# AUTOMATIC1111/stable-diffusion-webui

Hardware: AMD Instinct MI355X
Metric: images/sec SD1.5 512x512 20-step Euler-a, batch 8 per GPU (higher is better)
Workload: dtype f16

## Files before the change

include/sdmi.h:

```cpp
#ifndef SDMI_H
#define SDMI_H

#include <stdint.h>

#ifdef __cplusplus
extern "C" {
#endif

#define SDMI_VERSION 100

enum { SDMI_F16 = 0, SDMI_F32 = 1 };

typedef struct sdmi_engine sdmi_engine;

int sdmi_version(void);
const char* sdmi_last_error(void);
int sdmi_device_ok(void);


int64_t sdmi_attention_workspace_bytes(int B, int H, int M, int D);
int sdmi_attention(const void* q, const void* k, const void* v, void* out,
                   int B, int H, int N, int M, int D,
                   int ldq, int ldk, int ldv, int ldo, float scale,
                   void* workspace, int64_t workspace_bytes, void* stream);

int64_t sdmi_attention_wide_workspace_bytes(int B, int N, int M, int D);
int sdmi_attention_wide(const void* q, const void* k, const void* v, void* out,
                        int B, int N, int M, int D,
                        int ldq, int ldk, int ldv, int ldo, float scale,
                        void* workspace, int64_t workspace_bytes, void* stream);

int sdmi_attention_vt(const void* q, const void* k, const void* vt, void* out,
                      int B, int H, int N, int M, int D,
                      int ldq, int ldk, int vt_ld, int ldo, float scale, int force_generic, void* stream);

typedef struct sdmi_conv_desc {
    const void* a0;
    const void* a1;
    const void* w;
    const void* bias;
    const void* rowbias;
    const void* resid;
    void* out;
    int32_t c0, c1, lda0, lda1;
    int32_t B, Hi, Wi, Ho, Wo;
    int32_t taps;
    int32_t stride;
    int32_t pad;
    int32_t up;
// ... 323 lines not shown
```

stable-diffusion-webui_amd/_lib.py:

```python
from __future__ import annotations

import ctypes as C
import os
import re

_HERE = os.path.dirname(os.path.abspath(__file__))
LIB_PATH = os.environ.get("SDMI_LIB") or os.path.join(_HERE, "lib", "libsdmi.so")
HEADER_PATH = os.path.join(os.path.dirname(_HERE), "include", "sdmi.h")

F16, F32 = 0, 1
EP_OUT_F32, EP_GEGLU, EP_NCHW, EP_BIAS_ROW = 1, 2, 4, 8
EP_TRANSPOSE = 64
EP_WRAP = 128
RRDB_EP_NONE, RRDB_EP_LRELU, RRDB_EP_RES1, RRDB_EP_RES2, RRDB_EP_RELU = 0, 1, 2, 3, 4
RRDB_ST_F16, RRDB_ST_F32_NCHW, RRDB_ST_U8_HWC = 0, 1, 2
COMPACT_EP_NONE, COMPACT_EP_PRELU, COMPACT_EP_TAIL = 0, 1, 2


class SdmiError(RuntimeError):
    pass


class ConvDesc(C.Structure):
    _fields_ = [
# ... 86 lines not shown
        f"{LIB_PATH} is missing: build it with `python -c 'import __graft_entry__ as g; g.build()'` "
        "(hipcc --offload-arch=gfx950). There is no CPU fallback for the MI355X engine.")

lib = C.CDLL(LIB_PATH)

_vp, _i, _i64, _f, _u32 = C.c_void_p, C.c_int, C.c_int64, C.c_float, C.c_uint32
_SIGS = {
    "sdmi_version": (C.c_int, []),
    "sdmi_last_error": (C.c_char_p, []),
    "sdmi_device_ok": (C.c_int, []),
    "sdmi_attention_workspace_bytes": (_i64, [_i, _i, _i, _i]),
    "sdmi_attention": (_i, [_vp, _vp, _vp, _vp, _i, _i, _i, _i, _i, _i, _i, _i, _i, _f, _vp, _i64, _vp]),
    "sdmi_attention_wide_workspace_bytes": (_i64, [_i, _i, _i, _i]),
    "sdmi_attention_wide": (_i, [_vp, _vp, _vp, _vp, _i, _i, _i, _i, _i, _i, _i, _i, _f, _vp, _i64, _vp]),
    "sdmi_attention_vt": (_i, [_vp, _vp, _vp, _vp, _i, _i, _i, _i, _i, _i, _i, _i, _i, _f, _i, _vp]),
    "sdmi_conv_gemm": (_i, [C.POINTER(ConvDesc), _vp]),
    "sdmi_conv_splitk_workspace_bytes": (_i64, [_i, _i, _i, _i]),
    "sdmi_bench_conv_gemm": (_i, [C.POINTER(ConvDesc), _i, C.POINTER(C.c_float), _vp]),
    "sdmi_pack_conv_weight": (_i, [_vp, _i, _vp, _i, _i, _i, _i, _i, _i, _i, _vp]),
    "sdmi_groupnorm": (_i, [_vp, _vp, _i, _i, _vp, _vp, _vp, _i, _i, _i, _f, _i, _vp, _i64, _vp]),
    "sdmi_groupnorm_workspace_bytes": (_i64, [_i, _i, _i]),
    "sdmi_layernorm": (_i, [_vp, _vp, _vp, _vp, _i64, _i, _f, _vp]),
    "sdmi_rowchain_ff_pack_bytes": (_i64, [_i, _i]),
    "sdmi_rowchain_ff_pack": (_i, [_vp, _vp, _vp, _vp, _i, _i, _vp]),
    "sdmi_rowchain_ff": (_i, [_vp, _vp, _vp, _vp, _vp, _vp, _i64, _i, _i, _f, _vp]),
    "sdmi_xattn_chain": (_i, [_vp, _vp, _vp, _vp, _vp, _vp, _vp, _vp, _vp, _i64, _i, _i, _i, _i, _i, _f, _vp]),
    "sdmi_philox_randn": (_i, [_vp, _i64, C.c_uint64, C.c_uint32, _vp]),
    "sdmi_slerp": (_i, [_vp, _vp, _vp, _f, _i, _i, _i, _vp, _vp]),
    "sdmi_cfg_prepare_input": (_i, [_vp, _vp, _vp, _i, _i, _i, _i64, _vp]),
    "sdmi_cfg_prepare_concat": (_i, [_vp, _vp, _vp, _vp, _i, _i, _i, _i, _i, _i64, _u32, _vp]),
# ... 120 lines not shown
```

stable-diffusion-webui_amd/csrc/attention.hip:

```cpp
#include "common.h"
#include "prof.h"
#include <cstdlib>

namespace sdmi {

typedef float f2v __attribute__((ext_vector_type(2)));
typedef unsigned u4v __attribute__((ext_vector_type(4)));

__device__ __forceinline__ float max3f(float a, float b, float c) { return fmaxf(fmaxf(a, b), c); }
template <int NKB>
__device__ __forceinline__ float tree_max(const f16v (&sc)[NKB]) {
    constexpr int N = NKB * 16;
    float v[N];
#pragma unroll
    for (int i = 0; i < N; ++i) v[i] = sc[i >> 4][i & 15];
    int n = N;
#pragma unroll
    for (int level = 0; level < 6; ++level) {
        if (n <= 1) break;
        const int m = (n + 2) / 3;
#pragma unroll
        for (int i = 0; i < m; ++i) {
            const int a = 3 * i, b = a + 1 < n ? a + 1 : a, c = a + 2 < n ? a + 2 : a;
            v[i] = max3f(v[a], v[b], v[c]);
        }
        n = m;
    }
    return v[0];
}

__device__ __forceinline__ float fold_p2(float c) { return __builtin_bit_cast(float, __builtin_bit_cast(unsigned, c) & 0x7F800000u); }

template <int D, int KVT, int VAR = 0>
__global__ __launch_bounds__(256, ((VAR == 15 || VAR == 16 || VAR == 17 || VAR == 18) ? 3 : (VAR == 5 || VAR >= 10) ? 4 : D <= 80 ? 2 : 1)) void attn_mfma_kernel(AttnP p) {
    constexpr bool LAZY_RESCALE = VAR >= 5;
    constexpr bool PREF = VAR == 15 || VAR == 16 || VAR == 17 || VAR == 18;
    constexpr bool FOLD = VAR == 17 && ((D + 15) / 16 * 16) > D;
    constexpr bool TREEMAX = VAR == 16;
    constexpr bool TIMING = VAR == 18;
    long long tm[6] = {0, 0, 0, 0, 0, 0};
    auto stamp = [&]() -> long long {
        if constexpr (!TIMING) return 0;
        const long long t = __builtin_amdgcn_s_memtime();
        asm volatile("s_waitcnt lgkmcnt(0)" ::: "memory");
        return t;
    };
    constexpr bool NO_EXP = VAR == 10, NO_S = VAR == 11, NO_PV = VAR == 12, NO_MAX = VAR == 13, NO_STAGE = VAR == 14;
    constexpr int DK = (D + 15) / 16 * 16;
    constexpr int NDC = DK / 16;
    constexpr int DV = (D + 31) / 32 * 32;
    constexpr int NDB = DV / 32;
    constexpr int NKB = KVT / 32;
// ... 24 lines not shown
            bh = blockIdx.y; qb = blockIdx.x;
        }
    }
    const int b = bh / p.H, h = bh - b * p.H;
    const int q = qb * 128 + wave * 32 + lq;
    const bool qok = q < p.N;

    h8 qf[NDC];
    {
        const half_t* qptr = p.q + ((long)b * p.N + (qok ? q : 0)) * p.ldq + h * D;
#pragma unroll
        for (int dc = 0; dc < NDC; ++dc) {
            const int d = dc * 16 + half * 8;
            h8 v = {0, 0, 0, 0, 0, 0, 0, 0};
            if (qok && d < D) v = *reinterpret_cast<const h8*>(qptr + d);
            if constexpr (FOLD) {
#pragma unroll
                for (int e = 0; e < 8; ++e) v[e] = (half_t)((float)v[e] * fold_p2(p.scale_log2));
            }
            qf[dc] = v;
        }
    }
    constexpr int F_DC = D / 16, F_HALF = (D >> 3) & 1, F_E = D & 7;
    float shift = 0.f;

    const half_t* kbase = p.k + (long)b * p.M * p.ldk + h * D;
    const half_t* vbase = p.vt + ((long)b * p.H + h) * D * (long)p.vt_ld;

    u4v kr[K_IT], vr[V_IT];
    auto load_tile = [&](int t) {
        const int key0 = t * KVT;
#pragma unroll
        for (int it = 0; it < K_IT; ++it) {
            const int idx = it * 256 + tid;
            const int row = idx / KCPR, c = idx - row * KCPR;
            const int rr = min(key0 + row, p.M - 1);
            const int cc = (DK == D || c * 8 < D) ? c : 0;
            kr[it] = *reinterpret_cast<const u4v*>(kbase + (long)rr * p.ldk + cc * 8);
        }
#pragma unroll
        for (int it = 0; it < V_IT; ++it) {
            const int idx = it * 256 + tid;
            const int row = idx / VCPR, c = idx - row * VCPR;
            int col = key0 + c * 8;
            if (KVT > 64) col = min(col, p.vt_ld - 8);
            vr[it] = *reinterpret_cast<const u4v*>(vbase + (long)min(row, D - 1) * p.vt_ld + col);
        }
    };
    auto write_tile = [&](int buf) {
        char* Ks = smem + buf * TILE_BYTES;
        char* Vs = Ks + K_BYTES;
#pragma unroll
        for (int it = 0; it < K_IT; ++it) {
            const int idx = it * 256 + tid;
            const int row = idx / KCPR, c = idx - row * KCPR;
            if ((KCH % 256 == 0 || it + 1 < K_IT || idx < KCH) && !(FOLD && c * 8 >= D)) *reinterpret_cast<u4v*>(Ks + row * KSTR + c * 16) = kr[it];
        }
#pragma unroll
        for (int it = 0; it < V_IT; ++it) {
            const int idx = it * 256 + tid;
            const int row = idx / VCPR, c = idx - row * VCPR;
// ... 28 lines not shown
        constexpr int PADCH = (DV - D) * VCPR;
        for (int i = tid; i < 2 * PADCH; i += 256) {
            const int buf = i / PADCH, j = i - buf * PADCH;
            const int row = D + j / VCPR, c = j % VCPR;
            const unsigned w = row == D ? 0x3C003C00u : 0u;
            *reinterpret_cast<uint4*>(smem + buf * TILE_BYTES + K_BYTES + row * VSTR + c * 16) = make_uint4(w, w, w, w);
        }
    }
    __syncthreads();

    const f2v sl2 = {p.scale_log2, p.scale_log2};
    for (int t = 0; t < ntiles; ++t) {
        const int cur = t & 1;
        const bool more = !NO_STAGE && t + 1 < ntiles;
        const long long ta = stamp();
        if (more) load_tile(t + 1);
        const char* tile = smem + (NO_STAGE ? 0 : cur) * TILE_BYTES;

        f16v sc[NKB];
#pragma unroll
        for (int kb = 0; kb < NKB; ++kb)
#pragma unroll
            for (int r = 0; r < 16; ++r) sc[kb][r] = 0.f;
        h8 vaf[PREF ? NDB : 1][PREF ? NKB : 1][2];
        if constexpr (PREF) {
            h8 kaf[NDC][NKB];
#pragma unroll
            for (int dc = 0; dc < NDC; ++dc)
#pragma unroll
                for (int kb = 0; kb < NKB; ++kb) kaf[dc][kb] = *reinterpret_cast<const h8*>(tile + ka_off + kb * 32 * KSTR + dc * 32);
// ... 24 lines not shown

        const long long tb = stamp();
        if (t >= nfull || p.causal) {
            asm volatile("");
            int lim = p.M - t * KVT - 8 * half;
            if (p.causal) lim = min(lim, q + 1 - t * KVT - 8 * half);
#pragma unroll
            for (int kb = 0; kb < NKB; ++kb)
#pragma unroll
                for (int r = 0; r < 16; ++r)
                    if (32 * kb + 16 * (r >> 3) + (r & 7) >= lim) sc[kb][r] = -INFINITY;
        }
        h8 pb[NKB][2];
        long long tc = 0;
        if constexpr (FOLD) {
            const float fr = p.scale_log2 / fold_p2(p.scale_log2);
            const f2v fr2 = {fr, fr};
            float mx = -INFINITY;
#pragma unroll
            for (int kb = 0; kb < NKB; ++kb)
#pragma unroll
                for (int r = 0; r < 16; ++r) mx = fmaxf(mx, sc[kb][r]);
            float mlo = mx, mhi = mx;
            asm volatile("s_nop 1\n\tv_permlane32_swap_b32 %0, %1" : "+v"(mlo), "+v"(mhi));
            mx = fmaxf(mlo, mhi);
            const bool up = t == 0 || mx * fr > fmaxf(p.tau, 0.f);
            if (__builtin_amdgcn_ballot_w64(up) != 0) {
                asm volatile("");
                const float want = fmaxf(shift + mx, -60000.f);
                half_t hs = (half_t)want;
                float f = (float)hs;
                if (f < want) {
                    unsigned short bits = __builtin_bit_cast(unsigned short, hs);
                    bits = (f >= 0.f) ? (unsigned short)(bits + 1) : (unsigned short)(bits - 1);
                    hs = __builtin_bit_cast(half_t, bits);
                    f = (float)hs;
                }
                const float delta = up ? f - shift : 0.f;
                if (up) shift = f;
                const float alpha = __builtin_amdgcn_exp2f(-delta * fr);
#pragma unroll
                for (int kb = 0; kb < NKB; ++kb)
#pragma unroll
                    for (int r = 0; r < 16; ++r) sc[kb][r] -= delta;
#pragma unroll
                for (int db = 0; db < NDB; ++db)
#pragma unroll
                    for (int r = 0; r < 16; ++r) o[db][r] *= alpha;
                if (half == F_HALF) qf[F_DC][F_E] = (half_t)(-shift);
            }
#pragma unroll
            for (int kb = 0; kb < NKB; ++kb)
#pragma unroll
                for (int r = 0; r < 16; r += 2) {
                    const f2v y = f2v{sc[kb][r], sc[kb][r + 1]} * fr2;
                    pb[kb][r >> 3][r & 7] = (half_t)__builtin_amdgcn_exp2f(y.x);
                    pb[kb][r >> 3][(r & 7) + 1] = (half_t)__builtin_amdgcn_exp2f(y.y);
                }
        } else {
        float mx = -INFINITY;
        if constexpr (NO_MAX) { mx = sc[0][0] * p.scale_log2; }
        else {
        if constexpr (TREEMAX) mx = tree_max<NKB>(sc);
        else {
#pragma unroll
        for (int kb = 0; kb < NKB; ++kb)
#pragma unroll
            for (int r = 0; r < 16; ++r) mx = fmaxf(mx, sc[kb][r]);
        }
        if constexpr (PREF) {
// ... 532 lines not shown
}

template <int D, bool FOLD, int NG = 2, bool TIMING = false>
static int launch_attn_pp(const AttnP& p, hipStream_t s) {
    constexpr int DK = (D + 15) / 16 * 16, DV = (D + 31) / 32 * 32;
    constexpr int SMEM = 3 * (64 * (DK * 2 + 16) + DV * (64 * 2 + 16)) + 64 * (DK * 2 + 16) + NG * 256 * 16;
    auto kern = attn_pp_kernel<D, FOLD, NG, TIMING>;
    static PerDeviceOnce attr;
    if (attr.need()) SDMI_CHECK_HIP(hipFuncSetAttribute((const void*)kern, hipFuncAttributeMaxDynamicSharedMemorySize, SMEM));
    dim3 grid(cdiv(p.N, NG * 128), p.B * p.H);
    hipLaunchKernelGGL(kern, grid, dim3(NG * 256), SMEM, s, p);
    SDMI_CHECK_HIP(hipGetLastError());
    return 0;
}

int launch_attention(const AttnP& p_in, bool force_generic, hipStream_t s) {
    AttnP p = p_in;
    p.tau = (float)(g_attn_tau < 0 ? -1 : g_attn_tau > 12 ? 12 : g_attn_tau);
    SDMI_REQUIRE(p.B > 0 && p.H > 0 && p.N > 0 && p.M > 0 && p.D > 0, "empty attention");
    SDMI_REQUIRE(p.vt_ld >= (p.M + 63) / 64 * 64, "vt_ld must be >= M rounded up to 64");
    const double pf_flops = 4.0 * p.B * p.H * (double)p.N * p.M * p.D;
    const double pf_bytes = 2.0 * p.B * p.H * ((double)p.N * p.D * 2 + (double)p.M * p.D * 2);
    ProfScope ps(force_generic ? "attention_generic" : (p.M > 128 ? "attention_mfma_self" : "attention_mfma_cross"), pf_flops, pf_bytes, s);
    const bool aligned = (p.ldq % 8 == 0) && (p.ldk % 8 == 0) && (p.vt_ld % 8 == 0) && (p.ldo % 4 == 0) && (p.D % 8 == 0);
    const bool kvt128 = g_attn_kvt == 128;
    if (!force_generic && aligned) {
        if (g_attn_kvt == 96 && p.M > 64 && p.M <= 96 && !p.causal) {
            switch (p.D) {
                case 40: return launch_attn_d<40, 96, 0>(p, s);
                case 64: return launch_attn_d<64, 96>(p, s);
                case 80: return launch_attn_d<80, 96>(p, s);
                case 160: return launch_attn_d<160, 96>(p, s);
                default: break;
            }
        }
        switch (p.D) {
            case 40:
                if ((g_attn_occ == 20 || g_attn_occ == 21) && p.M >= g_attn_pp_min_m && p.N >= 256)
                    return g_attn_occ == 21 ? launch_attn_pp<40, true>(p, s) : launch_attn_pp<40, false>(p, s);
                if ((g_attn_occ == 28 || g_attn_occ == 38) && p.M >= g_attn_pp_min_m && p.N >= 384) {
                    AttnP q = p; q.dbg = (long long*)g_attn_dbg;
                    return g_attn_occ == 38 ? launch_attn_pp<40, true, 3, true>(q, s) : launch_attn_pp<40, true, 2, true>(q, s);
                }
                if ((g_attn_occ == 30 || g_attn_occ == 31) && p.M >= g_attn_pp_min_m && p.N >= 384)
                    return g_attn_occ == 31 ? launch_attn_pp<40, true, 3>(p, s) : launch_attn_pp<40, false, 3>(p, s);
                if (!(kvt128 && p.M > 64)) {
                    if (g_attn_occ == 5) return launch_attn_d<40, 64, 5>(p, s);
                    if (g_attn_occ == 15 && g_attn_fold_min_m > 0 && p.M >= g_attn_fold_min_m && p.N >= g_attn_fold_min_m && !p.causal)
                        return launch_attn_d<40, 64, 17>(p, s);
                    if (g_attn_occ == 15) return launch_attn_d<40, 64, 15>(p, s);
                    if (g_attn_occ == 16) return launch_attn_d<40, 64, 16>(p, s);
                    if (g_attn_occ == 17) return launch_attn_d<40, 64, 17>(p, s);
#ifdef SDMI_ATTN_PARTS
                    if (g_attn_occ == 10) return launch_attn_d<40, 64, 10>(p, s);
                    if (g_attn_occ == 11) return launch_attn_d<40, 64, 11>(p, s);
                    if (g_attn_occ == 12) return launch_attn_d<40, 64, 12>(p, s);
                    if (g_attn_occ == 13) return launch_attn_d<40, 64, 13>(p, s);
                    if (g_attn_occ == 14) return launch_attn_d<40, 64, 14>(p, s);
                    if (g_attn_occ == 18) { AttnP q = p; q.dbg = (long long*)g_attn_dbg; return launch_attn_d<40, 64, 18>(q, s); }
#endif
                }
                return (kvt128 && p.M > 64) ? launch_attn_d<40, 128>(p, s) : launch_attn_d<40, 64>(p, s);
            case 64:
                if ((g_attn_occ == 20 || g_attn_occ == 21) && p.M >= g_attn_pp_min_m && p.N >= 256) return launch_attn_pp<64, false>(p, s);
                return (kvt128 && p.M > 64) ? launch_attn_d<64, 128>(p, s) : launch_attn_d<64, 64>(p, s);
            case 80: return launch_attn_d<80, 64>(p, s);
            case 128: return launch_attn_d<128, 64>(p, s);
            case 160: return launch_attn_d<160, 64>(p, s);
            default: break;
        }
    }
    SDMI_REQUIRE(p.D <= 512 && p.M <= 16384, "generic attention supports D <= 512 and M <= 16384");
    static PerDeviceOnce attr;
    if (attr.need()) SDMI_CHECK_HIP(hipFuncSetAttribute((const void*)attn_generic_kernel, hipFuncAttributeMaxDynamicSharedMemorySize, 16384 * 4));
    hipLaunchKernelGGL(attn_generic_kernel, dim3(p.N, p.B * p.H), dim3(64), p.M * sizeof(float), s, p);
    SDMI_CHECK_HIP(hipGetLastError());
    return 0;
}

// ... 2 lines not shown
```

stable-diffusion-webui_amd/csrc/capi.cpp:

```cpp
#include "engine.h"
#include "prof.h"
#include <cstring>

namespace sdmi {
extern int g_vae_attn_rows;
int unet_forward(sdmi_engine* e, const void* x, const void* t, const void* ctx, const void* y, void* out, int io_dtype,
                 int Bn, int h, int w, int L, hipStream_t s);
int vae_decode(sdmi_engine* e, const void* z, int io_dtype, float* out, int B, int h, int w, hipStream_t s);
int vae_encode(sdmi_engine* e, const void* x, int io_dtype, float* out, int B, int H, int W, hipStream_t s);
int engine_load_unet_tensor(sdmi_engine* e, const char* key, const void* data, int dtype, int ndim, const int64_t* shape, int on_device);
int engine_load_vae_tensor(sdmi_engine* e, const char* key, const void* data, int dtype, int ndim, const int64_t* shape, int on_device);
int engine_unet_finalize(sdmi_engine* e);
int engine_clip_configure(sdmi_engine* e, int slot, const sdmi_clip_config* cfg);
int engine_clip_load_tensor(sdmi_engine* e, int slot, const char* key, const void* data, int dtype, int ndim, const int64_t* shape, int on_device);
int engine_clip_finalize(sdmi_engine* e, int slot);
int engine_clip_forward(sdmi_engine* e, int slot, const int* tokens, const float* inputs_embeds, int B, int L, int skip,
                        int apply_final_ln, float* out, float* pooled, hipStream_t s);
int engine_unet_update_weight(sdmi_engine* e, const char* key, const void* data, int dtype, int ndim, const int64_t* shape, int on_device);
int engine_vae_finalize(sdmi_engine* e);
int engine_hypernet_clear(sdmi_engine* e);
int engine_hypernet_begin(sdmi_engine* e, float multiplier);
int engine_hypernet_linear(sdmi_engine* e, int dim, int which, const void* w, const void* b, int dtype, int out_f, int in_f, int on_device);
int engine_hypernet_act(sdmi_engine* e, int dim, int which, int act);
int engine_hypernet_layernorm(sdmi_engine* e, int dim, int which, const void* g, const void* b, int dtype, int n, int on_device);
// ... 48 lines not shown
    const int64_t mpad = (M + 63) / 64 * 64;
    return (int64_t)B * H * D * mpad * (int64_t)sizeof(half_t);
}

int sdmi_attention_vt(const void* q, const void* k, const void* vt, void* out, int B, int H, int N, int M, int D, int ldq,
                      int ldk, int vt_ld, int ldo, float scale, int force_generic, void* stream) {
    API_GUARD_BEGIN
    AttnP p{};
    p.q = (const half_t*)q; p.k = (const half_t*)k; p.vt = (const half_t*)vt; p.out = (half_t*)out;
    p.B = B; p.H = H; p.N = N; p.M = M; p.D = D; p.ldq = ldq; p.ldk = ldk; p.vt_ld = vt_ld; p.ldo = ldo;
    p.scale_log2 = scale * 1.4426950408889634f;
    return launch_attention(p, force_generic != 0, (hipStream_t)stream);
    API_GUARD_END
}

int sdmi_attention(const void* q, const void* k, const void* v, void* out, int B, int H, int N, int M, int D, int ldq,
                   int ldk, int ldv, int ldo, float scale, void* workspace, int64_t workspace_bytes, void* stream) {
    API_GUARD_BEGIN
    SDMI_REQUIRE(workspace && workspace_bytes >= sdmi_attention_workspace_bytes(B, H, M, D), "attention workspace too small");
    const int mpad = (M + 63) / 64 * 64;
    if (launch_transpose_v((const half_t*)v, (half_t*)workspace, B, H, M, D, ldv, mpad, (hipStream_t)stream)) return 1;
    return sdmi_attention_vt(q, k, workspace, out, B, H, N, M, D, ldq, ldk, mpad, ldo, scale, 0, stream);
    API_GUARD_END
}

static constexpr int kWideRows = 4096;
int64_t sdmi_attention_wide_workspace_bytes(int B, int N, int M, int D) {
    if (B <= 0 || N <= 0 || M <= 0 || D <= 0) return 0;
    const int64_t mpad = (M + 63) / 64 * 64;
    const int64_t rows = N < kWideRows ? N : kWideRows;
// ... 677 lines not shown
    else if (n == "vae_attn_rows") g_vae_attn_rows = value;
    else if (n == "gemm_shortk_maxk") g_shortk_max_k = value;
    else if (n == "gemm_geglu_cfg") g_geglu_gemm_cfg = value;
    else if (n == "vt_mode") g_vt_mode = value;
    else if (n == "tile_order") g_tile_order = value;
    else if (n == "conv_korder") g_conv_korder = value < 0 ? g_conv_korder_default : value;
    else if (n == "small_linear_lds") g_small_linear_lds = value;
    else if (n == "gn_fuse") g_gn_fuse = value;
    else if (n == "gn_small") g_gn_small = value;
    else if (n == "ep_wide") g_ep_wide = value;
    else if (n == "attn_kvt") g_attn_kvt = value;
    else if (n == "attn_occ") g_attn_occ = value;
    else if (n == "attn_lds_pad") g_attn_lds_pad = value;
    else if (n == "attn_fold_min_m") g_attn_fold_min_m = value;
    else if (n == "attn_tau") g_attn_tau = value;
    else if (n == "attn_dbg_lo") g_attn_dbg = (g_attn_dbg & 0xFFFFFFFF00000000ull) | (unsigned)value;
    else if (n == "attn_dbg_hi") g_attn_dbg = (g_attn_dbg & 0xFFFFFFFFull) | ((unsigned long long)(unsigned)value << 32);
    else if (n == "gemm_split") g_force_gemm_split = value;
    else if (n == "gemm_pipe") g_gemm_pipe = value < 0 ? g_gemm_pipe_default : value;
    else if (n == "gemm_lin") g_gemm_lin = value < 0 ? 1 : value;
    else if (n == "gn_apply_blocks") g_gn_apply_blocks = value < 0 ? 0 : value;
    else if (n == "gn_band_elems") g_gn_band_elems = value < 0 ? 0 : value;
    else if (n == "gemm_dbgflags") g_gemm_dbgflags = value & 0x1F00;
    else if (n == "gemm_dbg_lo") g_gemm_dbg = (g_gemm_dbg & 0xFFFFFFFF00000000ull) | (unsigned)value;
    else if (n == "gemm_dbg_hi") g_gemm_dbg = (g_gemm_dbg & 0xFFFFFFFFull) | ((unsigned long long)(unsigned)value << 32);
    else { set_error("unknown debug knob " + n); return 1; }
    return 0;
    API_GUARD_END
}

// ... 73 lines not shown
```

stable-diffusion-webui_amd/csrc/common.h:

```cpp
#pragma once
#include <hip/hip_runtime.h>
#include <stdint.h>
#include <string>

typedef _Float16 half_t;
typedef _Float16 h8 __attribute__((ext_vector_type(8)));
typedef _Float16 h4 __attribute__((ext_vector_type(4)));
typedef _Float16 h2 __attribute__((ext_vector_type(2)));
typedef float f4 __attribute__((ext_vector_type(4)));
typedef float f16v __attribute__((ext_vector_type(16)));

namespace sdmi {

#ifndef SDMI_GELU_SIG
#define SDMI_GELU_SIG 1
#endif
__device__ __forceinline__ float geglu_gate(float val, float g) {
    const float gc = fminf(fmaxf(g, -10.0f), 10.0f);
    const float g2 = gc * gc;
    float p = fmaf(1.01426306e-3f, g2, -0.106775724f);
    p = fmaf(p, g2, -2.30112135f);
    const float e = __builtin_amdgcn_exp2f(p * gc);
    return (val * g) * __builtin_amdgcn_rcpf(1.0f + e);
}
// ... 108 lines not shown
extern int g_conv_korder;
extern int g_conv_korder_default;
extern int g_tile_order;
extern int g_vt_mode;
extern long g_gn_band_elems;
extern int g_gn_apply_blocks;
extern int g_gemm_lin;
extern int g_gemm_pipe;
extern int g_gemm_pipe_default;
extern int g_force_gemm_split;
extern int g_attn_kvt;
extern int g_attn_occ;
extern int g_attn_lds_pad;
extern int g_attn_fold_min_m;
extern int g_attn_tau;
extern unsigned long long g_attn_dbg;
extern int g_gemm_dbgflags;
extern unsigned long long g_gemm_dbg;

struct AttnP {
    const half_t* q;
    const half_t* k;
    const half_t* vt;
    half_t* out;
    int B, H, N, M, D;
    int ldq, ldk, vt_ld, ldo;
    float scale_log2;
    int causal;
    long long* dbg;
    float tau;
};
int launch_attention(const AttnP& p, bool force_generic, hipStream_t s);
int launch_transpose_v(const half_t* v, half_t* vt, int B, int H, int M, int D, int ldv, int Mpad, hipStream_t s);

bool rowchain_supports(int C);
size_t rowchain_ff_pack_bytes(int C, int hidden);
int launch_rowchain_ff_pack(const half_t* w1, const float* b1, const half_t* w2, void* packs, int C, int hidden, bool permuted,
                            hipStream_t s);
int launch_rowchain_ff(const half_t* x, half_t* out, const float* gamma, const float* beta, const void* packs, const float* bias_out,
                       long rows, int C, int hidden, float eps, hipStream_t s);

int launch_xattn_chain(const half_t* x, half_t* out, const float* gamma, const float* beta, const half_t* wq, const half_t* wo,
                       const float* bo, const half_t* k, const half_t* vt, long rows, int rows_per_image, int C, int heads, int L, int Lpad,
                       float eps, hipStream_t s);

enum { RRDB_EP_NONE = 0, RRDB_EP_LRELU = 1,
       RRDB_EP_RES1 = 2,
// ... 154 lines not shown
```

stable-diffusion-webui_amd/csrc/engine.cpp:

```cpp
#include "engine.h"

#include <algorithm>
#include <cmath>
#include <cstring>
#include <functional>

namespace sdmi {

static thread_local std::string g_err;
void set_error(const std::string& m) { g_err = m; }
const char* get_error() { return g_err.c_str(); }

const half_t* zero_page() {
    static thread_local int cached_dev = -1;
    static thread_local half_t* cached = nullptr;
    static std::map<int, half_t*> pages;
    int dev = 0;
    if (hipGetDevice(&dev) != hipSuccess) return nullptr;
    if (dev == cached_dev) return cached;
    auto it = pages.find(dev);
    if (it == pages.end()) {
        void* p = nullptr;
        if (hipMalloc(&p, kZeroPageHalfs * sizeof(half_t)) != hipSuccess) return nullptr;
        if (hipMemset(p, 0, kZeroPageHalfs * sizeof(half_t)) != hipSuccess) return nullptr;
// ... 511 lines not shown
        ConvArgs c;
        c.a0 = t2; c.c0 = w.cout; c.B = B; c.Hi = H; c.Wi = Wd; c.Ho = H; c.Wo = Wd; c.pad = 1;
        c.resid = resid; c.ldr = w.cout; c.out = o; c.ldo = w.cout;
        c.resid_lo = resid_lo; c.out_lo = acc ? r.lo(o, (out_buf ? LR : M) * w.cout) : nullptr;
        c.alpha = ss; c.bias_scale = ss;
        c.stats_C = ss == 1.f ? w.cout : 0;
        c.stats_ws_pre = st_pre;
        TRY(run_conv(r, w.c2, c));
    }
    if (reuse) r.ar->rewind(mk);
    *out = o;
    return 0;
}

static int run_attn(Run& r, const half_t* q, const half_t* k, const half_t* vt, half_t* out, int B, int H, int N, int M,
                    int D, int ldq, int ldk, int vt_ld, int ldo) {
    if (r.dry) return 0;
    AttnP p{};
    p.q = q; p.k = k; p.vt = vt; p.out = out;
    p.B = B; p.H = H; p.N = N; p.M = M; p.D = D;
    p.ldq = ldq; p.ldk = ldk; p.vt_ld = vt_ld; p.ldo = ldo;
    p.scale_log2 = (1.0f / sqrtf((float)D)) * 1.4426950408889634f;
    return launch_attention(p, r.e->force_generic, r.s);
}

static int run_vt(Run& r, const ConvW& Wv, const half_t* x, int ldx, int B, int tokens, int tokens_pad, half_t* vt,
                  bool bias_row, const int* gate = nullptr) {
    if (r.dry) return 0;
    GemmP p{};
    const int C = Wv.n_pad, K = Wv.cin_pad;
    if (g_vt_mode == 1 && tokens == tokens_pad && tokens % 4 == 0 && ldx == K && gate == nullptr) {
        p.a0 = x; p.c0 = K; p.cin = K; p.lda0 = ldx;
        p.w = Wv.w; p.ldw = K;
        p.bias = bias_row ? Wv.b : nullptr;
        p.out = vt;
        p.Hi = tokens; p.Wi = 1; p.Ho = tokens; p.Wo = 1;
        p.taps = 1; p.stride = 1; p.pad = 0; p.up = 0;
        p.M = B * tokens; p.N = C; p.K = K; p.n_valid = C;
// ... 98 lines not shown
        if (fold) {
            LnStats st1;
            TRY(run_ln_stats(r, b.ln1, cur, M, &st1));
            half_t* qk = r.H(M * 2 * C);
            TRY(run_linear_ln(r, b.qk1, b.ln1, cur, st1, (int)M, qk, 2 * C));
            half_t* vt = r.H((size_t)B * C * Npad);
            TRY(run_vt_ln(r, b.v1, b.ln1, cur, st1, B, HW, Npad, vt));
            a1 = r.H(M * C);
            TRY(run_attn(r, qk, qk + C, vt, a1, B, st.heads, HW, HW, st.dhead, 2 * C, 2 * C, Npad, C));
        }
        half_t* n1 = fold ? nullptr : r.H(M * C);
        if (!fold) TRY(run_ln(r, b.ln1, cur, M1, n1, r.lo(cur, MC)));
        if (fold) {
        } else if (!hn_has_dim(e, C)) {
            half_t* qk = r.H(M * 2 * C);
            TRY(run_linear(r, b.qk1, n1, (int)M1, nullptr, qk, 2 * C));
            half_t* vt = r.H((size_t)B * C * Npad);
            TRY(run_vt(r, b.v1, n1, C, B1, HW, Npad, vt, false));
            a1 = r.H(M * C);
            TRY(run_attn(r, qk, qk + C, vt, a1, B1, st.heads, HW, HW, st.dhead, 2 * C, 2 * C, Npad, C));
        } else {
            auto alloc = [&](size_t n) { return r.H(n); };
            const half_t *xk = nullptr, *xv = nullptr;
            TRY(run_hn(r, C, 0, n1, M, alloc, false, &xk));
            TRY(run_hn(r, C, 1, n1, M, alloc, false, &xv));
            ConvW wq = b.qk1, wk = b.qk1;
            wq.n_pad = wk.n_pad = C; wq.cout = wk.cout = C;
            wk.w = b.qk1.w + (size_t)C * b.qk1.cin_pad;
            if (b.qk1.b) wk.b = b.qk1.b + C;
            half_t* q = r.H(M * C);
            half_t* k = r.H(M * C);
            TRY(run_linear(r, wq, n1, (int)M, nullptr, q, C));
            TRY(run_linear(r, wk, xk, (int)M, nullptr, k, C));
            half_t* vt = r.H((size_t)B * C * Npad);
            TRY(run_vt(r, b.v1, xv, C, B, HW, Npad, vt, false));
// ... 1910 lines not shown
```

stable-diffusion-webui_amd/ops.py:

```python
from __future__ import annotations

import ctypes as C
from typing import Optional

import torch

from . import _lib
from ._lib import lib, check, ptr, stream_ptr, ConvDesc, F16, F32, EP_OUT_F32, EP_GEGLU, EP_NCHW, EP_BIAS_ROW


def _rup(x, m):
    return (x + m - 1) // m * m


def attention(q: torch.Tensor, k: torch.Tensor, v: torch.Tensor, heads: int, scale: Optional[float] = None) -> torch.Tensor:
    _lib.require_device()
    assert q.dtype == torch.float16 and k.dtype == torch.float16 and v.dtype == torch.float16
    b, n, c = q.shape
    m = k.shape[1]
    d = c // heads
    q, k, v = [t if t.stride(-1) == 1 and t.stride(0) == t.shape[1] * t.stride(1) else t.contiguous() for t in (q, k, v)]
    out = torch.empty((b, n, c), dtype=torch.float16, device=q.device)
    scale = d ** -0.5 if scale is None else scale
    if heads == 1 and d > 160 and d % 64 == 0:
# ... 4 lines not shown
        return out
    ws_bytes = lib.sdmi_attention_workspace_bytes(b, heads, m, d)
    ws = torch.empty(ws_bytes, dtype=torch.uint8, device=q.device)
    check(lib.sdmi_attention(ptr(q), ptr(k), ptr(v), ptr(out), b, heads, n, m, d, q.stride(1), k.stride(1), v.stride(1),
                             out.stride(1), float(scale), ptr(ws), ws_bytes, stream_ptr()), "sdmi_attention")
    return out


def attention_vt(q, k, vt, heads, m, scale=None, force_generic=False):
    b, n, c = q.shape
    d = c // heads
    out = torch.empty((b, n, c), dtype=torch.float16, device=q.device)
    scale = d ** -0.5 if scale is None else scale
    check(lib.sdmi_attention_vt(ptr(q), ptr(k), ptr(vt), ptr(out), b, heads, n, m, d, q.stride(1), k.stride(1), vt.shape[2],
                                out.stride(1), float(scale), 1 if force_generic else 0, stream_ptr()), "sdmi_attention_vt")
    return out


def pack_conv_weight(w: torch.Tensor, geglu: bool = False, pad: int = 64) -> torch.Tensor:
    _lib.require_device()
    w = w.contiguous()
    if w.dim() == 2:
        w = w[:, :, None, None]
    o, i, kh, kw = w.shape
    o_pad, i_pad = _rup(o, pad), _rup(i, pad)
    out = torch.empty((o_pad, kh * kw, i_pad), dtype=torch.float16, device=w.device)
    check(lib.sdmi_pack_conv_weight(ptr(w), _lib.dtype_code(w), ptr(out), o, i, kh, kw, o_pad, i_pad, 1 if geglu else 0,
                                    stream_ptr()), "pack_conv_weight")
    return out

# ... 358 lines not shown
```

Measured before the change: 20.71.

## Fold attention softmax scale into QK projection and precompute tile load offsets

Adds an attention form (27) for head dim 40 that takes q and k already scaled by sqrt(scale*log2e), applied in the fused QK projection epilogue. This removes the per-score multiply and the q fold rescale inside the flash kernel. The same form precomputes 32-bit per-thread byte offsets for K and V^T tile loads, so the inner loop spends less address arithmetic. It is gated on an env default of on, no QK bias, no fp32 residual, and the engine's attn_occ/fold settings. Scaling q and k in f16 before the dot product slightly changes rounding.

```diff
diff --git a/include/sdmi.h b/include/sdmi.h
--- a/include/sdmi.h
+++ b/include/sdmi.h
@@ -33,6 +33,10 @@
 int sdmi_attention_vt(const void* q, const void* k, const void* vt, void* out,
                       int B, int H, int N, int M, int D,
                       int ldq, int ldk, int vt_ld, int ldo, float scale, int force_generic, void* stream);
+
+int sdmi_attention_vt_ex(const void* q, const void* k, const void* vt, void* out,
+                         int B, int H, int N, int M, int D,
+                         int ldq, int ldk, int vt_ld, int ldo, float scale, int prescaled, int form, int force_generic, void* stream);
 
 typedef struct sdmi_conv_desc {
     const void* a0;
diff --git a/stable-diffusion-webui_amd/_lib.py b/stable-diffusion-webui_amd/_lib.py
--- a/stable-diffusion-webui_amd/_lib.py
+++ b/stable-diffusion-webui_amd/_lib.py
@@ -124,6 +124,7 @@
     "sdmi_attention_wide_workspace_bytes": (_i64, [_i, _i, _i, _i]),
     "sdmi_attention_wide": (_i, [_vp, _vp, _vp, _vp, _i, _i, _i, _i, _i, _i, _i, _i, _f, _vp, _i64, _vp]),
     "sdmi_attention_vt": (_i, [_vp, _vp, _vp, _vp, _i, _i, _i, _i, _i, _i, _i, _i, _i, _f, _i, _vp]),
+    "sdmi_attention_vt_ex": (_i, [_vp, _vp, _vp, _vp, _i, _i, _i, _i, _i, _i, _i, _i, _i, _f, _i, _i, _i, _vp]),
     "sdmi_conv_gemm": (_i, [C.POINTER(ConvDesc), _vp]),
     "sdmi_conv_splitk_workspace_bytes": (_i64, [_i, _i, _i, _i]),
     "sdmi_bench_conv_gemm": (_i, [C.POINTER(ConvDesc), _i, C.POINTER(C.c_float), _vp]),
diff --git a/stable-diffusion-webui_amd/csrc/attention.hip b/stable-diffusion-webui_amd/csrc/attention.hip
--- a/stable-diffusion-webui_amd/csrc/attention.hip
+++ b/stable-diffusion-webui_amd/csrc/attention.hip
@@ -32,10 +32,13 @@
 __device__ __forceinline__ float fold_p2(float c) { return __builtin_bit_cast(float, __builtin_bit_cast(unsigned, c) & 0x7F800000u); }
 
 template <int D, int KVT, int VAR = 0>
-__global__ __launch_bounds__(256, ((VAR == 15 || VAR == 16 || VAR == 17 || VAR == 18) ? 3 : (VAR == 5 || VAR >= 10) ? 4 : D <= 80 ? 2 : 1)) void attn_mfma_kernel(AttnP p) {
+__global__ __launch_bounds__(256, ((VAR == 15 || VAR == 16 || VAR == 17 || VAR == 18 || VAR == 27) ? 3 : (VAR == 5 || VAR >= 10) ? 4 : D <= 80 ? 2 : 1)) void attn_mfma_kernel(AttnP p) {
     constexpr bool LAZY_RESCALE = VAR >= 5;
-    constexpr bool PREF = VAR == 15 || VAR == 16 || VAR == 17 || VAR == 18;
-    constexpr bool FOLD = VAR == 17 && ((D + 15) / 16 * 16) > D;
+    constexpr bool STAGE = VAR == 27;
+    constexpr bool PRESC = VAR == 27;
+    constexpr bool PREF = VAR == 15 || VAR == 16 || VAR == 17 || VAR == 18 || STAGE;
+    constexpr bool FOLD = (VAR == 17 || STAGE) && ((D + 15) / 16 * 16) > D;
+    static_assert(!STAGE || (FOLD && KVT == 64), "form 27: folded shift, 64-key tiles (no V^T column clamp)");
     constexpr bool TREEMAX = VAR == 16;
     constexpr bool TIMING = VAR == 18;
     long long tm[6] = {0, 0, 0, 0, 0, 0};
@@ -90,7 +93,7 @@
             const int d = dc * 16 + half * 8;
             h8 v = {0, 0, 0, 0, 0, 0, 0, 0};
             if (qok && d < D) v = *reinterpret_cast<const h8*>(qptr + d);
-            if constexpr (FOLD) {
+            if constexpr (FOLD && !PRESC) {
 #pragma unroll
                 for (int e = 0; e < 8; ++e) v[e] = (half_t)((float)v[e] * fold_p2(p.scale_log2));
             }
@@ -121,6 +124,38 @@
             int col = key0 + c * 8;
             if (KVT > 64) col = min(col, p.vt_ld - 8);
             vr[it] = *reinterpret_cast<const u4v*>(vbase + (long)min(row, D - 1) * p.vt_ld + col);
+        }
+    };
+    [[maybe_unused]] unsigned koff[STAGE ? K_IT : 1], voff[STAGE ? V_IT : 1];
+    if constexpr (STAGE) {
+#pragma unroll
+        for (int it = 0; it < K_IT; ++it) {
+            const int idx = it * 256 + tid;
+            const int row = idx / KCPR, c = idx - row * KCPR;
+            const int cc = (DK == D || c * 8 < D) ? c : 0;
+            koff[it] = (unsigned)(min(row, KVT - 1) * p.ldk + cc * 8) * 2u;
+        }
+#pragma unroll
+        for (int it = 0; it < V_IT; ++it) {
+            const int idx = it * 256 + tid;
+            const int row = idx / VCPR, c = idx - row * VCPR;
+            voff[it] = (unsigned)(min(row, D - 1) * p.vt_ld + c * 8) * 2u;
+        }
+    }
+    auto load_full_tile = [&](int t) {
+        if constexpr (STAGE) {
+            const char* kt = reinterpret_cast<const char*>(kbase) + (long)t * KVT * p.ldk * 2;
+            const char* vt = reinterpret_cast<const char*>(vbase) + (long)t * KVT * 2;
+#pragma unroll
+            for (int it = 0; it < K_IT; ++it) {
+                asm volatile("" : "+v"(koff[it]));
+                kr[it] = *reinterpret_cast<const u4v*>(kt + koff[it]);
+            }
+#pragma unroll
+            for (int it = 0; it < V_IT; ++it) {
+                asm volatile("" : "+v"(voff[it]));
+                vr[it] = *reinterpret_cast<const u4v*>(vt + voff[it]);
+            }
         }
     };
     auto write_tile = [&](int buf) {
@@ -179,6 +214,10 @@
         const int cur = t & 1;
         const bool more = !NO_STAGE && t + 1 < ntiles;
         const long long ta = stamp();
+        if constexpr (STAGE) {
+            if (t + 1 < nfull) load_full_tile(t + 1);
+            else if (more) load_tile(t + 1);
+        } else
         if (more) load_tile(t + 1);
         const char* tile = smem + (NO_STAGE ? 0 : cur) * TILE_BYTES;
 
@@ -233,7 +272,7 @@
         h8 pb[NKB][2];
         long long tc = 0;
         if constexpr (FOLD) {
-            const float fr = p.scale_log2 / fold_p2(p.scale_log2);
+            const float fr = PRESC ? 1.f : p.scale_log2 / fold_p2(p.scale_log2);
             const f2v fr2 = {fr, fr};
             float mx = -INFINITY;
 #pragma unroll
@@ -243,7 +282,9 @@
             float mlo = mx, mhi = mx;
             asm volatile("s_nop 1\n\tv_permlane32_swap_b32 %0, %1" : "+v"(mlo), "+v"(mhi));
             mx = fmaxf(mlo, mhi);
-            const bool up = t == 0 || mx * fr > fmaxf(p.tau, 0.f);
+            bool up;
+            if constexpr (PRESC) up = t == 0 || mx > fmaxf(p.tau, 0.f);
+            else up = t == 0 || mx * fr > fmaxf(p.tau, 0.f);
             if (__builtin_amdgcn_ballot_w64(up) != 0) {
                 asm volatile("");
                 const float want = fmaxf(shift + mx, -60000.f);
@@ -257,7 +298,9 @@
                 }
                 const float delta = up ? f - shift : 0.f;
                 if (up) shift = f;
-                const float alpha = __builtin_amdgcn_exp2f(-delta * fr);
+                float alpha;
+                if constexpr (PRESC) alpha = __builtin_amdgcn_exp2f(-delta);
+                else alpha = __builtin_amdgcn_exp2f(-delta * fr);
 #pragma unroll
                 for (int kb = 0; kb < NKB; ++kb)
 #pragma unroll
@@ -272,7 +315,8 @@
             for (int kb = 0; kb < NKB; ++kb)
 #pragma unroll
                 for (int r = 0; r < 16; r += 2) {
-                    const f2v y = f2v{sc[kb][r], sc[kb][r + 1]} * fr2;
+                    f2v y = f2v{sc[kb][r], sc[kb][r + 1]};
+                    if constexpr (!PRESC) y = y * fr2;
                     pb[kb][r >> 3][r & 7] = (half_t)__builtin_amdgcn_exp2f(y.x);
                     pb[kb][r >> 3][(r & 7) + 1] = (half_t)__builtin_amdgcn_exp2f(y.y);
                 }
@@ -835,15 +879,34 @@
     return 0;
 }
 
+int g_attn_prescale = [] { const char* e = getenv("SDMI_ATTN_PRESCALE"); return e ? atoi(e) : 1; }();
+
+static bool attn_stage_fits(const AttnP& p) {
+    return 64.0 * p.ldk * 2 < 2147483648.0 && (double)p.D * p.vt_ld * 2 < 2147483648.0;
+}
+static bool attn_aligned(const AttnP& p) {
+    return (p.ldq % 8 == 0) && (p.ldk % 8 == 0) && (p.vt_ld % 8 == 0) && (p.ldo % 4 == 0) && (p.D % 8 == 0);
+}
+
+bool attn_takes_prescaled(const AttnP& p, bool force_generic) {
+    if (force_generic || !attn_aligned(p) || p.D != 40 || p.causal || g_attn_kvt == 128 || g_attn_kvt == 96) return false;
+    if (!g_attn_prescale || !attn_stage_fits(p)) return false;
+    if (g_attn_occ == 27) return true;
+    return g_attn_occ == 15 && g_attn_fold_min_m > 0 && p.M >= g_attn_fold_min_m && p.N >= g_attn_fold_min_m;
+}
+
 int launch_attention(const AttnP& p_in, bool force_generic, hipStream_t s) {
     AttnP p = p_in;
+    const bool pre = p.prescaled != 0;
+    const int occ = p.form > 0 ? p.form : g_attn_occ;
+    if (pre) p.scale_log2 = 1.f;
     p.tau = (float)(g_attn_tau < 0 ? -1 : g_attn_tau > 12 ? 12 : g_attn_tau);
     SDMI_REQUIRE(p.B > 0 && p.H > 0 && p.N > 0 && p.M > 0 && p.D > 0, "empty attention");
     SDMI_REQUIRE(p.vt_ld >= (p.M + 63) / 64 * 64, "vt_ld must be >= M rounded up to 64");
     const double pf_flops = 4.0 * p.B * p.H * (double)p.N * p.M * p.D;
     const double pf_bytes = 2.0 * p.B * p.H * ((double)p.N * p.D * 2 + (double)p.M * p.D * 2);
     ProfScope ps(force_generic ? "attention_generic" : (p.M > 128 ? "attention_mfma_self" : "attention_mfma_cross"), pf_flops, pf_bytes, s);
-    const bool aligned = (p.ldq % 8 == 0) && (p.ldk % 8 == 0) && (p.vt_ld % 8 == 0) && (p.ldo % 4 == 0) && (p.D % 8 == 0);
+    const bool aligned = attn_aligned(p);
     const bool kvt128 = g_attn_kvt == 128;
     if (!force_generic && aligned) {
         if (g_attn_kvt == 96 && p.M > 64 && p.M <= 96 && !p.causal) {
@@ -857,33 +920,42 @@
         }
         switch (p.D) {
             case 40:
-                if ((g_attn_occ == 20 || g_attn_occ == 21) && p.M >= g_attn_pp_min_m && p.N >= 256)
-                    return g_attn_occ == 21 ? launch_attn_pp<40, true>(p, s) : launch_attn_pp<40, false>(p, s);
-                if ((g_attn_occ == 28 || g_attn_occ == 38) && p.M >= g_attn_pp_min_m && p.N >= 384) {
+                if ((occ == 20 || occ == 21) && p.M >= g_attn_pp_min_m && p.N >= 256)
+                    return occ == 21 ? launch_attn_pp<40, true>(p, s) : launch_attn_pp<40, false>(p, s);
+                if ((occ == 28 || occ == 38) && p.M >= g_attn_pp_min_m && p.N >= 384) {
                     AttnP q = p; q.dbg = (long long*)g_attn_dbg;
-                    return g_attn_occ == 38 ? launch_attn_pp<40, true, 3, true>(q, s) : launch_attn_pp<40, true, 2, true>(q, s);
+                    return occ == 38 ? launch_attn_pp<40, true, 3, true>(q, s) : launch_attn_pp<40, true, 2, true>(q, s);
                 }
-                if ((g_attn_occ == 30 || g_attn_occ == 31) && p.M >= g_attn_pp_min_m && p.N >= 384)
-                    return g_attn_occ == 31 ? launch_attn_pp<40, true, 3>(p, s) : launch_attn_pp<40, false, 3>(p, s);
+                if ((occ == 30 || occ == 31) && p.M >= g_attn_pp_min_m && p.N >= 384)
+                    return occ == 31 ? launch_attn_pp<40, true, 3>(p, s) : launch_attn_pp<40, false, 3>(p, s);
                 if (!(kvt128 && p.M > 64)) {
-                    if (g_attn_occ == 5) return launch_attn_d<40, 64, 5>(p, s);
-                    if (g_attn_occ == 15 && g_attn_fold_min_m > 0 && p.M >= g_attn_fold_min_m && p.N >= g_attn_fold_min_m && !p.causal)
+                    if (occ == 5) return launch_attn_d<40, 64, 5>(p, s);
+                    if (occ == 15 && g_attn_fold_min_m > 0 && p.M >= g_attn_fold_min_m && p.N >= g_attn_fold_min_m && !p.causal) {
+                        if (pre && attn_stage_fits(p)) return launch_attn_d<40, 64, 27>(p, s);
                         return launch_attn_d<40, 64, 17>(p, s);
-                    if (g_attn_occ == 15) return launch_attn_d<40, 64, 15>(p, s);
-                    if (g_attn_occ == 16) return launch_attn_d<40, 64, 16>(p, s);
-                    if (g_attn_occ == 17) return launch_attn_d<40, 64, 17>(p, s);
+                    }
+                    if (occ == 15) return launch_attn_d<40, 64, 15>(p, s);
+                    if (occ == 16) return launch_attn_d<40, 64, 16>(p, s);
+                    if (occ == 17) return launch_attn_d<40, 64, 17>(p, s);
+                    if (occ == 27) {
+                        if (p.form == 27) {
+                            SDMI_REQUIRE(pre, "attention form 27 takes pre-scaled q and k only");
+                            SDMI_REQUIRE(attn_stage_fits(p), "attention form 27: a tile's byte offsets must fit 32 bits");
+                        }
+                        return (pre && attn_stage_fits(p)) ? launch_attn_d<40, 64, 27>(p, s) : launch_attn_d<40, 64, 17>(p, s);
+                    }
 #ifdef SDMI_ATTN_PARTS
-                    if (g_attn_occ == 10) return launch_attn_d<40, 64, 10>(p, s);
-                    if (g_attn_occ == 11) return launch_attn_d<40, 64, 11>(p, s);
-                    if (g_attn_occ == 12) return launch_attn_d<40, 64, 12>(p, s);
-                    if (g_attn_occ == 13) return launch_attn_d<40, 64, 13>(p, s);
-                    if (g_attn_occ == 14) return launch_attn_d<40, 64, 14>(p, s);
-                    if (g_attn_occ == 18) { AttnP q = p; q.dbg = (long long*)g_attn_dbg; return launch_attn_d<40, 64, 18>(q, s); }
+                    if (occ == 10) return launch_attn_d<40, 64, 10>(p, s);
+                    if (occ == 11) return launch_attn_d<40, 64, 11>(p, s);
+                    if (occ == 12) return launch_attn_d<40, 64, 12>(p, s);
+                    if (occ == 13) return launch_attn_d<40, 64, 13>(p, s);
+                    if (occ == 14) return launch_attn_d<40, 64, 14>(p, s);
+                    if (occ == 18) { AttnP q = p; q.dbg = (long long*)g_attn_dbg; return launch_attn_d<40, 64, 18>(q, s); }
 #endif
                 }
                 return (kvt128 && p.M > 64) ? launch_attn_d<40, 128>(p, s) : launch_attn_d<40, 64>(p, s);
             case 64:
-                if ((g_attn_occ == 20 || g_attn_occ == 21) && p.M >= g_attn_pp_min_m && p.N >= 256) return launch_attn_pp<64, false>(p, s);
+                if ((occ == 20 || occ == 21) && p.M >= g_attn_pp_min_m && p.N >= 256) return launch_attn_pp<64, false>(p, s);
                 return (kvt128 && p.M > 64) ? launch_attn_d<64, 128>(p, s) : launch_attn_d<64, 64>(p, s);
             case 80: return launch_attn_d<80, 64>(p, s);
             case 128: return launch_attn_d<128, 64>(p, s);
diff --git a/stable-diffusion-webui_amd/csrc/capi.cpp b/stable-diffusion-webui_amd/csrc/capi.cpp
--- a/stable-diffusion-webui_amd/csrc/capi.cpp
+++ b/stable-diffusion-webui_amd/csrc/capi.cpp
@@ -86,6 +86,20 @@
     API_GUARD_END
 }
 
+int sdmi_attention_vt_ex(const void* q, const void* k, const void* vt, void* out, int B, int H, int N, int M, int D, int ldq,
+                         int ldk, int vt_ld, int ldo, float scale, int prescaled, int form, int force_generic, void* stream) {
+    API_GUARD_BEGIN
+    AttnP p{};
+    p.q = (const half_t*)q; p.k = (const half_t*)k; p.vt = (const half_t*)vt; p.out = (half_t*)out;
+    p.B = B; p.H = H; p.N = N; p.M = M; p.D = D; p.ldq = ldq; p.ldk = ldk; p.vt_ld = vt_ld; p.ldo = ldo;
+    p.scale_log2 = scale * 1.4426950408889634f;
+    p.prescaled = prescaled != 0;
+    SDMI_REQUIRE(form >= 0 && form < 100, "form: an attn_occ value");
+    p.form = (short)form;
+    return launch_attention(p, force_generic != 0, (hipStream_t)stream);
+    API_GUARD_END
+}
+
 int sdmi_attention(const void* q, const void* k, const void* v, void* out, int B, int H, int N, int M, int D, int ldq,
                    int ldk, int ldv, int ldo, float scale, void* workspace, int64_t workspace_bytes, void* stream) {
     API_GUARD_BEGIN
@@ -793,6 +807,7 @@
     else if (n == "attn_lds_pad") g_attn_lds_pad = value;
     else if (n == "attn_fold_min_m") g_attn_fold_min_m = value;
     else if (n == "attn_tau") g_attn_tau = value;
+    else if (n == "attn_prescale") g_attn_prescale = value < 0 ? 1 : value;
     else if (n == "attn_dbg_lo") g_attn_dbg = (g_attn_dbg & 0xFFFFFFFF00000000ull) | (unsigned)value;
     else if (n == "attn_dbg_hi") g_attn_dbg = (g_attn_dbg & 0xFFFFFFFFull) | ((unsigned long long)(unsigned)value << 32);
     else if (n == "gemm_split") g_force_gemm_split = value;
diff --git a/stable-diffusion-webui_amd/csrc/common.h b/stable-diffusion-webui_amd/csrc/common.h
--- a/stable-diffusion-webui_amd/csrc/common.h
+++ b/stable-diffusion-webui_amd/csrc/common.h
@@ -146,6 +146,7 @@
 extern int g_attn_lds_pad;
 extern int g_attn_fold_min_m;
 extern int g_attn_tau;
+extern int g_attn_prescale;
 extern unsigned long long g_attn_dbg;
 extern int g_gemm_dbgflags;
 extern unsigned long long g_gemm_dbg;
@@ -161,8 +162,11 @@
     int causal;
     long long* dbg;
     float tau;
+    short form;
+    short prescaled;
 };
 int launch_attention(const AttnP& p, bool force_generic, hipStream_t s);
+bool attn_takes_prescaled(const AttnP& p, bool force_generic);
 int launch_transpose_v(const half_t* v, half_t* vt, int B, int H, int M, int D, int ldv, int Mpad, hipStream_t s);
 
 bool rowchain_supports(int C);
diff --git a/stable-diffusion-webui_amd/csrc/engine.cpp b/stable-diffusion-webui_amd/csrc/engine.cpp
--- a/stable-diffusion-webui_amd/csrc/engine.cpp
+++ b/stable-diffusion-webui_amd/csrc/engine.cpp
@@ -549,14 +549,22 @@
 }
 
 static int run_attn(Run& r, const half_t* q, const half_t* k, const half_t* vt, half_t* out, int B, int H, int N, int M,
-                    int D, int ldq, int ldk, int vt_ld, int ldo) {
+                    int D, int ldq, int ldk, int vt_ld, int ldo, bool prescaled = false) {
     if (r.dry) return 0;
     AttnP p{};
     p.q = q; p.k = k; p.vt = vt; p.out = out;
     p.B = B; p.H = H; p.N = N; p.M = M; p.D = D;
     p.ldq = ldq; p.ldk = ldk; p.vt_ld = vt_ld; p.ldo = ldo;
     p.scale_log2 = (1.0f / sqrtf((float)D)) * 1.4426950408889634f;
+    p.prescaled = prescaled;
     return launch_attention(p, r.e->force_generic, r.s);
+}
+static bool attn_prescale_ok(const Run& r, const ConvW& qk, int B, int H, int N, int D, int ld, int vt_ld, int ldo) {
+    if (qk.b != nullptr || r.e->residual_fp32) return false;
+    AttnP p{};
+    p.B = B; p.H = H; p.N = N; p.M = N; p.D = D;
+    p.ldq = ld; p.ldk = ld; p.vt_ld = vt_ld; p.ldo = ldo;
+    return attn_takes_prescaled(p, r.e->force_generic);
 }
 
 static int run_vt(Run& r, const ConvW& Wv, const half_t* x, int ldx, int B, int tokens, int tokens_pad, half_t* vt,
@@ -685,11 +693,13 @@
         if (fold) {
         } else if (!hn_has_dim(e, C)) {
             half_t* qk = r.H(M * 2 * C);
-            TRY(run_linear(r, b.qk1, n1, (int)M1, nullptr, qk, 2 * C));
+            const bool pre = attn_prescale_ok(r, b.qk1, B1, st.heads, HW, st.dhead, 2 * C, Npad, C);
+            const float qk_ss = pre ? sqrtf((1.0f / sqrtf((float)st.dhead)) * 1.4426950408889634f) : 1.f;
+            TRY(run_linear(r, b.qk1, n1, (int)M1, nullptr, qk, 2 * C, qk_ss));
             half_t* vt = r.H((size_t)B * C * Npad);
             TRY(run_vt(r, b.v1, n1, C, B1, HW, Npad, vt, false));
             a1 = r.H(M * C);
-            TRY(run_attn(r, qk, qk + C, vt, a1, B1, st.heads, HW, HW, st.dhead, 2 * C, 2 * C, Npad, C));
+            TRY(run_attn(r, qk, qk + C, vt, a1, B1, st.heads, HW, HW, st.dhead, 2 * C, 2 * C, Npad, C, pre));
         } else {
             auto alloc = [&](size_t n) { return r.H(n); };
             const half_t *xk = nullptr, *xv = nullptr;
diff --git a/stable-diffusion-webui_amd/ops.py b/stable-diffusion-webui_amd/ops.py
--- a/stable-diffusion-webui_amd/ops.py
+++ b/stable-diffusion-webui_amd/ops.py
@@ -42,6 +42,17 @@
     scale = d ** -0.5 if scale is None else scale
     check(lib.sdmi_attention_vt(ptr(q), ptr(k), ptr(vt), ptr(out), b, heads, n, m, d, q.stride(1), k.stride(1), vt.shape[2],
                                 out.stride(1), float(scale), 1 if force_generic else 0, stream_ptr()), "sdmi_attention_vt")
+    return out
+
+
+def attention_vt_ex(q, k, vt, heads, m, scale=None, prescaled=False, form=0, force_generic=False):
+    b, n, _ = q.shape
+    d = vt.shape[1] // heads
+    out = torch.empty((b, n, heads * d), dtype=torch.float16, device=q.device)
+    scale = d ** -0.5 if scale is None else scale
+    check(lib.sdmi_attention_vt_ex(ptr(q), ptr(k), ptr(vt), ptr(out), b, heads, n, m, d, q.stride(1), k.stride(1), vt.shape[2],
+                                   out.stride(1), float(scale), 1 if prescaled else 0, int(form), 1 if force_generic else 0, stream_ptr()),
+          "sdmi_attention_vt_ex")
     return out
 
 
```

After: 21.02, median of 6. 1.01x the previous value.
